# Genie-Kim/PintheMemory

Measured on NVIDIA B200. Metric: memory read+update fwd+bwd Mpixels/s, higher is better.
Workload: dtype f32

## Files before the change

### pinthememory_b200/csrc/pm_gemm.cu

```cuda
#include "pm_common.cuh"
#include "pm_umma.cuh"

namespace pm {

constexpr int GEMM_THREADS = 320;
constexpr int GEMM_RING_BYTES = 192 * 1024;
constexpr int TILE_A_BYTES = 128 * 128;

template <typename T>
struct GemmTraits;
template <>
struct GemmTraits<float> {
    static constexpr int PXC = 32;
    static constexpr int UK = 8;
    static constexpr uint32_t FMT = UMMA_FMT_TF32;
    static constexpr bool SPLIT = true;
};
template <>
struct GemmTraits<__nv_bfloat16> {
    static constexpr int PXC = 64;
    static constexpr int UK = 16;
    static constexpr uint32_t FMT = UMMA_FMT_BF16;
    static constexpr bool SPLIT = false;
};

template <typename T>
__device__ __forceinline__ void umma_issue(uint32_t d, uint64_t a, uint64_t b, uint32_t idesc, uint32_t acc) {
    if constexpr (sizeof(T) == 4) umma_tf32(d, a, b, idesc, acc);
    else umma_bf16(d, a, b, idesc, acc);
}

__device__ __forceinline__ void split_tile_trunc(const float4* __restrict__ raw, float4* __restrict__ lo, int n4, int t,
                                                 int nthreads) {
    for (int i = t; i < n4; i += nthreads) {
        const float4 v = raw[i];
        float4 l;
        l.x = v.x - __uint_as_float(__float_as_uint(v.x) & 0xffffe000u);
        l.y = v.y - __uint_as_float(__float_as_uint(v.y) & 0xffffe000u);
        l.z = v.z - __uint_as_float(__float_as_uint(v.z) & 0xffffe000u);
        l.w = v.w - __uint_as_float(__float_as_uint(v.w) & 0xffffe000u);
        lo[i] = l;
    }
}
__device__ __forceinline__ uint32_t pack_bf16(float a, float b) {
    const __nv_bfloat162 p = __floats2bfloat162_rn(a, b);
    return *reinterpret_cast<const uint32_t*>(&p);
}
__device__ __forceinline__ float tf32_resid(float x) { return x - __uint_as_float(__float_as_uint(x) & 0xffffe000u); }

template <int KB, int NT>
__device__ __forceinline__ void mix_tile_mn(const unsigned char* __restrict__ raw, unsigned char* __restrict__ out, int t,
                                            int nthreads) {
    constexpr int NC32 = NT / 32, ATOMS = KB * NC32 * 4;
    for (int i = t; i < ATOMS; i += nthreads) {
// ... 23 lines not shown
        lo.x = pack_bf16(tf32_resid(v0.x), tf32_resid(v0.y)), lo.y = pack_bf16(tf32_resid(v0.z), tf32_resid(v0.w));
        lo.z = pack_bf16(tf32_resid(v1.x), tf32_resid(v1.y)), lo.w = pack_bf16(tf32_resid(v1.z), tf32_resid(v1.w));
        unsigned char* ro = out + r * 128;
        const int jh = hi_first ? m : 4 + m, jl = hi_first ? 4 + m : m;
        *reinterpret_cast<uint4*>(ro + ((jh ^ (r & 7)) << 4)) = hi;
        *reinterpret_cast<uint4*>(ro + ((jl ^ (r & 7)) << 4)) = lo;
    }
}

__device__ __forceinline__ float tf32_rn(float x) { return __uint_as_float((__float_as_uint(x) + 0x00001000u) & 0xffffe000u); }
__device__ __forceinline__ void split_tile(float4* __restrict__ raw, float4* __restrict__ lo, int n4, int t, int nthreads) {
    for (int i = t; i < n4; i += nthreads) {
        const float4 v = raw[i];
        float4 h, l;
        h.x = tf32_rn(v.x), h.y = tf32_rn(v.y), h.z = tf32_rn(v.z), h.w = tf32_rn(v.w);
        l.x = v.x - h.x, l.y = v.y - h.y, l.z = v.z - h.z, l.w = v.w - h.w;
        lo[i] = l;
        raw[i] = h;
    }
}

struct BnBwdArgs {
    const float *mean, *invstd, *gamma, *beta, *dgamma, *dbeta;
    float inv_n;
    int training, relu;
};

template <int KB>
__device__ __forceinline__ void bnbwd_tile(float4* __restrict__ dy_hi, float4* __restrict__ z_lo, int n4, int t, int nthreads,
                                           int ch0, const BnBwdArgs& bn) {
    constexpr bool FIXED = (KB == 16);
    float is = 0.f, mu = 0.f, sc = 0.f, sh = 0.f, k1 = 0.f, k2 = 0.f;
    auto coef = [&](int c) {
        is = __ldg(bn.invstd + c), mu = __ldg(bn.mean + c);
        sc = is * __ldg(bn.gamma + c), sh = __ldg(bn.beta + c) - mu * sc;
        k1 = bn.training ? __ldg(bn.dbeta + c) * bn.inv_n : 0.f, k2 = bn.training ? __ldg(bn.dgamma + c) * bn.inv_n : 0.f;
    };
    if (FIXED) coef(ch0 + ((t >> 3) % KB));
    for (int i = t; i < n4; i += nthreads) {
        if (!FIXED) coef(ch0 + ((i >> 3) % KB));
        const float4 g = dy_hi[i], z = z_lo[i];
        float4 d, l;
#define PM_BNBWD_ONE(f)                                                                  \
        {                                                                                \
            const float gv = (!bn.relu || fmaf(z.f, sc, sh) > 0.f) ? g.f : 0.f;          \
            const float xh = (z.f - mu) * is;                                            \
            d.f = sc * (gv - k1 - xh * k2);                                              \
            l.f = d.f - __uint_as_float(__float_as_uint(d.f) & 0xffffe000u);             \
        }
        PM_BNBWD_ONE(x) PM_BNBWD_ONE(y) PM_BNBWD_ONE(z) PM_BNBWD_ONE(w)
#undef PM_BNBWD_ONE
        dy_hi[i] = d;
        z_lo[i] = l;
    }
}

template <typename T, int MT, int NT, int KB, int CL, bool MIX>
__global__ void __launch_bounds__(GEMM_THREADS, 1)
    conv1x1_nn_kernel(const __grid_constant__ CUtensorMap mapX, const __grid_constant__ CUtensorMap mapAh,
                      const __grid_constant__ CUtensorMap mapAl, const __grid_constant__ CUtensorMap mapY, int K, int M,
                      int m_tile0, int tiles_per_img, int total_tiles, int accumulate, double* __restrict__ stats,
                      const float* __restrict__ ep_scale, const float* __restrict__ ep_shift, int ep_relu, int dbg,
                      const __grid_constant__ CUtensorMap mapZ, const __grid_constant__ CUtensorMap mapDZ, const BnBwdArgs bn) {
    using TR = GemmTraits<T>;
    constexpr int PXC = TR::PXC, UK = TR::UK, KSTEPS = KB / UK;
    const bool bnbwd = TR::SPLIT && !MIX && bn.mean != nullptr;
    constexpr int NCH = NT / PXC;
    constexpr int XCHUNK = KB * 128;
    constexpr int XBYTES = NCH * XCHUNK;
    constexpr int NOPA = TR::SPLIT ? 2 : 1;
    constexpr int AROW = KB * (int)sizeof(T);
    static_assert(AROW == 128 || AROW == 64, "weight rows must be 64 or 128 bytes");
    constexpr int TILE_A = 128 * AROW;
    constexpr uint32_t ASWZ = AROW == 128 ? UMMA_SW128 : UMMA_SW64, ASBO = 8 * AROW;
    constexpr int STAGE = NOPA * (XBYTES + MT * TILE_A);
    constexpr int STAGES = (GEMM_RING_BYTES / STAGE) > 4 ? 4 : (GEMM_RING_BYTES / STAGE);
    constexpr int ACC = (512 / (MT * NT)) >= 2 ? 2 : 1;
    constexpr uint32_t TX = XBYTES + NOPA * MT * TILE_A;
    static_assert(STAGES >= 2, "ring too small");
    static_assert(MT * NT <= 512, "accumulators exceed TMEM");
    constexpr uint32_t IDESC = umma_idesc(TR::FMT, false, true, 128, NT);
    constexpr uint32_t IDESC_B = umma_idesc(UMMA_FMT_BF16, false, true, 128, NT);
    static_assert(!MIX || (TR::SPLIT && KB % 16 == 0 && NT % 64 == 0), "mixed compensation: fp32 I/O, 16-channel groups");

    extern __shared__ unsigned char smem_raw[];
    unsigned char* smem = smem_align(smem_raw, 1024);
    unsigned char* stg = smem + STAGES * STAGE;
    uint64_t* bars = reinterpret_cast<uint64_t*>(stg + 4 * 2 * 4096);
    uint64_t* full = bars;
    uint64_t* empty = bars + STAGES;
    uint64_t* xfull = bars + 2 * STAGES;
    uint64_t* accf = bars + 3 * STAGES;
    uint64_t* acce = accf + ACC;
    uint64_t* sfree = acce + ACC;
    uint32_t* tmem_slot = reinterpret_cast<uint32_t*>(sfree + STAGES);

    const int warp = threadIdx.x >> 5, lane = threadIdx.x & 31;
    if (threadIdx.x == 0) {
        for (int i = 0; i < STAGES; ++i) {
            mbar_init(&full[i], 1);
            mbar_init(&empty[i], CL);
            mbar_init(&xfull[i], 4);
            mbar_init(&sfree[i], 1);
        }
        for (int i = 0; i < ACC; ++i) {
            mbar_init(&accf[i], 1);
// ... 79 lines not shown
                            const uint64_t ah = umma_desc(sa + mt * TILE_A + ks * 32, 16, ASBO, ASWZ);
                            if (MIX) {
                                umma_issue<T>(d, ah, bh, IDESC, first);
                            } else if (TR::SPLIT) {
                                const uint64_t al = umma_desc(sa + (MT + mt) * TILE_A + ks * 32, 16, ASBO, ASWZ);
                                umma_issue<T>(d, al, bh, IDESC, first);
                                umma_issue<T>(d, ah, bl, IDESC, 1u);
                                umma_issue<T>(d, ah, bh, IDESC, 1u);
                            } else {
                                umma_issue<T>(d, ah, bh, IDESC, first);
                            }
                        }
                    }
                    if (MIX) {
                        const int ksb = 2 * ksteps * UK / 16;
                        for (int ks = 0; ks < ksb; ++ks) {
                            const uint64_t bb = umma_desc(sx + XBYTES + ks * (16 * 128), 2 * KB * 128, 1024, UMMA_SW128);
#pragma unroll
                            for (int mt = 0; mt < MT; ++mt) {
                                const uint32_t d = tmem + (uint32_t)((a * MT + mt) * NT);
                                const uint64_t ab = umma_desc(sa + (MT + mt) * TILE_A + ks * 32, 16, ASBO, ASWZ);
                                umma_bf16(d, ab, bb, IDESC_B, 1u);
                            }
                        }
                    }
                    if (CL == 1) umma_commit(&empty[s]);
                    else umma_commit_multicast(&empty[s], (uint16_t)((1u << CL) - 1));
                }
                umma_commit(&accf[a]);
            }
        }
    } else if (warp < 6) {
        const int q = warp & 3;
        unsigned char* mystg = stg + q * 2 * 4096;
        int bi = 0;
        double sum[MT], sq[MT];
#pragma unroll
        for (int mt = 0; mt < MT; ++mt) sum[mt] = 0.0, sq[mt] = 0.0;
        uint32_t tc = 0;
        for (int g = g0; g < ngroups; g += gstride, ++tc) {
            const int tile = g * CL + crank;
            const int b = tile / tiles_per_img, px0 = (tile - b * tiles_per_img) * NT;
            const int a = tc % ACC;
            mbar_wait(&accf[a], (tc / ACC) & 1);
            tc_fence_after();
#pragma unroll
            for (int mt = 0; mt < MT; ++mt) {
                const int row0 = (m_tile0 + mt) * 128 + q * 32;
                if (row0 >= M || tile >= total_tiles) continue;
                const float sc = ep_scale != nullptr ? __ldg(ep_scale + row0 + lane) : 1.f;
                const float sh = ep_scale != nullptr ? __ldg(ep_shift + row0 + lane) : 0.f;
                float ts = 0.f, tq = 0.f;
                const uint32_t ta0 = tmem + ((uint32_t)(q * 32) << 16) + (uint32_t)((a * MT + mt) * NT);
                auto emit = [&](const uint4 (&out)[8], int c) {
                    unsigned char* buf = mystg + bi * 4096;
                    bi ^= 1;
                    if (lane == 0) bulk_wait_read<1>();
                    __syncwarp();
#pragma unroll
                    for (int j = 0; j < 8; ++j)
                        *reinterpret_cast<uint4*>(buf + lane * 128 + ((j ^ (lane & 7)) << 4)) = out[j];
                    fence_proxy_async_smem();
                    __syncwarp();
                    if (lane == 0) {
                        if (accumulate) tma_reduce_add_2d(&mapY, px0 + c * PXC, b * M + row0, buf);
                        else tma_store_2d(&mapY, px0 + c * PXC, b * M + row0, buf);
                        bulk_commit();
                    }
                };
                if constexpr (sizeof(T) == 4) {
                    auto process = [&](uint32_t (&r)[32], int c) {
                        if (ep_scale != nullptr) {
#pragma unroll
                            for (int j = 0; j < 32; ++j) {
                                float v = fmaf(__uint_as_float(r[j]), sc, sh);
                                if (ep_relu) v = fmaxf(v, 0.f);
                                r[j] = __float_as_uint(v);
                            }
                        }
#pragma unroll
                        for (int j = 0; j < 32; ++j) {
                            const float v = __uint_as_float(r[j]);
                            ts += v;
                            tq = fmaf(v, v, tq);
                        }
                        uint4 out[8];
#pragma unroll
                        for (int j = 0; j < 8; ++j) out[j] = make_uint4(r[4 * j], r[4 * j + 1], r[4 * j + 2], r[4 * j + 3]);
                        emit(out, c);
                    };
                    uint32_t ra[32], rb[32];
                    tmem_ld32(ta0, ra);
#pragma unroll 1
                    for (int c = 0; c < NCH; c += 2) {
                        tmem_ld_wait();
                        if (c + 1 < NCH) tmem_ld32(ta0 + (uint32_t)((c + 1) * PXC), rb);
                        process(ra, c);
                        if (c + 1 < NCH) {
                            tmem_ld_wait();
                            if (c + 2 < NCH) tmem_ld32(ta0 + (uint32_t)((c + 2) * PXC), ra);
                            process(rb, c + 1);
                        }
                    }
                } else {
#pragma unroll 1
                    for (int c = 0; c < NCH; ++c) {
                        const uint32_t ta = ta0 + (uint32_t)(c * PXC);
                        uint4 out[8];
                        uint32_t r0[32], r1[32];
                        tmem_ld32(ta, r0);
                        tmem_ld32(ta + 32, r1);
                        tmem_ld_wait();
                        if (ep_scale != nullptr) {
#pragma unroll
                            for (int j = 0; j < 32; ++j) {
                                float v0 = fmaf(__uint_as_float(r0[j]), sc, sh), v1 = fmaf(__uint_as_float(r1[j]), sc, sh);
                                if (ep_relu) v0 = fmaxf(v0, 0.f), v1 = fmaxf(v1, 0.f);
                                r0[j] = __float_as_uint(v0), r1[j] = __float_as_uint(v1);
                            }
                        }
                        uint32_t pk[32];
#pragma unroll
                        for (int j = 0; j < 16; ++j) {
                            const __nv_bfloat162 p0 = __floats2bfloat162_rn(__uint_as_float(r0[2 * j]), __uint_as_float(r0[2 * j + 1]));
                            const __nv_bfloat162 p1 = __floats2bfloat162_rn(__uint_as_float(r1[2 * j]), __uint_as_float(r1[2 * j + 1]));
                            pk[j] = *reinterpret_cast<const uint32_t*>(&p0);
                            pk[16 + j] = *reinterpret_cast<const uint32_t*>(&p1);
                            const float2 f0 = __bfloat1622float2(p0), f1 = __bfloat1622float2(p1);
                            ts += (f0.x + f0.y) + (f1.x + f1.y);
                            tq = fmaf(f0.x, f0.x, fmaf(f0.y, f0.y, fmaf(f1.x, f1.x, fmaf(f1.y, f1.y, tq))));
                        }
#pragma unroll
                        for (int j = 0; j < 8; ++j) out[j] = make_uint4(pk[4 * j], pk[4 * j + 1], pk[4 * j + 2], pk[4 * j + 3]);
                        emit(out, c);
                    }
                }
                sum[mt] += (double)ts;
                sq[mt] += (double)tq;
            }
            tc_fence_before();
            mbar_arrive(&acce[a]);
        }
        if (lane == 0) bulk_wait<0>();
        if (stats != nullptr) {
#pragma unroll
            for (int mt = 0; mt < MT; ++mt) {
                const int row = (m_tile0 + mt) * 128 + q * 32 + lane;
                if (row < M) {
                    atomicAdd(&stats[row], sum[mt]);
                    atomicAdd(&stats[M + row], sq[mt]);
                }
            }
        }
    } else {
        if constexpr (TR::SPLIT) {
            const int t = threadIdx.x - 6 * 32;
            uint32_t it = 0;
            for (int g = g0; g < ngroups; g += gstride) {
                int tile = g * CL + crank;
                const bool real_tile = tile < total_tiles;
                if (!real_tile) tile = total_tiles - 1;
                const int b = tile / tiles_per_img, px0 = (tile - b * tiles_per_img) * NT;
                for (int kb = 0; kb < nkb; ++kb, ++it) {
                    const int s = it % STAGES;
                    mbar_wait(&full[s], (it / STAGES) & 1);
                    unsigned char* st = smem + s * STAGE;
                    if (MIX) mix_tile_mn<KB, NT>(st, st + XBYTES, t, 128);
                    else if (bnbwd) bnbwd_tile<KB>(reinterpret_cast<float4*>(st), reinterpret_cast<float4*>(st + XBYTES), XBYTES / 16, t, 128, kb * KB, bn);
                    else split_tile_trunc(reinterpret_cast<float4*>(st), reinterpret_cast<float4*>(st + XBYTES), XBYTES / 16, t, 128);
                    fence_proxy_async_smem();
                    __syncwarp();
                    if (lane == 0) mbar_arrive(&xfull[s]);
                    if (bnbwd && t == 0) {
                        mbar_wait(&xfull[s], (it / STAGES) & 1);
                        if (real_tile) {
#pragma unroll
                            for (int c = 0; c < NCH; ++c) tma_store_2d(&mapDZ, px0 + c * PXC, b * K + kb * KB, st + c * XCHUNK);
                        }
                        bulk_commit();
                        bulk_wait_read<1>();
                        if (it > 0) mbar_arrive(&sfree[(it - 1) % STAGES]);
                    }
                }
            }
            if (bnbwd && t == 0) bulk_wait<0>();
        }
    }
// ... 69 lines not shown
    if (!make_map_2d<T>(&mX, X, (size_t)B * K, hw, KB, TR::PXC, sizeof(T) == 4 ? 2 : 1)) return PM_ERR_ALIGN;
    if (!make_map_2d<T>(&mAh, Ah, Mpad, K, 128, KB, ASW)) return PM_ERR_ALIGN;
    const bool mix = TR::SPLIT && gemm_mix() && K % 16 == 0 && bn.mean == nullptr;
    if (mix) {
        if (!make_map_2d<__nv_bfloat16>(&mAl, Al, Mpad, 2 * (size_t)K, 128, 2 * KB, ASW)) return PM_ERR_ALIGN;
    } else if (TR::SPLIT) {
        if (!make_map_2d<T>(&mAl, Al, Mpad, K, 128, KB, ASW)) return PM_ERR_ALIGN;
    } else {
        mAl = mAh;
    }
    if (!make_map_2d<T>(&mY, Y, (size_t)B * M, hw, 32, TR::PXC, true)) return PM_ERR_ALIGN;
    if (bn.mean == nullptr) mZ = mX, mDZ = mX;
    const int tiles_per_img = (hw + NT - 1) / NT, total = B * tiles_per_img;
    const size_t smem = nn_smem_bytes<T, MT, NT, KB>();
    constexpr int NBLK = (TR::SPLIT ? 2 : 1) * MT;
    constexpr int CLMAX = NBLK >= 4 ? 4 : NBLK;
    int cl = gemm_cluster();
    if (cl > CLMAX) cl = CLMAX;
    if (total < 2 * cl) cl = 1;
    cudaLaunchConfig_t cfg{};
    cudaLaunchAttribute attr[1];
    cfg.blockDim = dim3(GEMM_THREADS);
    cfg.dynamicSmemBytes = smem;
    cfg.stream = st;
    attr[0].id = cudaLaunchAttributeClusterDimension;
    attr[0].val.clusterDim.x = cl, attr[0].val.clusterDim.y = 1, attr[0].val.clusterDim.z = 1;
    cfg.attrs = attr, cfg.numAttrs = 1;
    int groups = (total + cl - 1) / cl, clusters = 148 / cl;
    if (clusters > groups) clusters = groups;
    cfg.gridDim = dim3(clusters * cl);
    const int dbg = gemm_dbg();
    cudaError_t e;
#define PM_NN_LAUNCH(CL_)                                                                                             \
    {                                                                                                                 \
        auto kern = mix ? conv1x1_nn_kernel<T, MT, NT, KB, CL_, TR::SPLIT> : conv1x1_nn_kernel<T, MT, NT, KB, CL_, false>; \
        e = cudaFuncSetAttribute(kern, cudaFuncAttributeMaxDynamicSharedMemorySize, (int)smem);                       \
        if (e != cudaSuccess) return (int)e;                                                                          \
        e = cudaLaunchKernelEx(&cfg, kern, mX, mAh, mAl, mY, K, M, m_tile0, tiles_per_img, total, accumulate, stats,     \
                               ep_scale, ep_shift, ep_relu, dbg, mZ, mDZ, bn);                                   \
    }
    if (cl == 4) {
        if constexpr (CLMAX >= 4) PM_NN_LAUNCH(4) else return PM_ERR_SHAPE;
    } else if (cl == 2) {
        if constexpr (CLMAX >= 2) PM_NN_LAUNCH(2) else return PM_ERR_SHAPE;
    } else {
        PM_NN_LAUNCH(1)
    }
#undef PM_NN_LAUNCH
    if (e != cudaSuccess) return (int)e;
    e = cudaGetLastError();
    return e == cudaSuccess ? 0 : (int)e;
}

constexpr int WG_NMAX = 288;

template <typename T, bool MIX>
__global__ void __launch_bounds__(GEMM_THREADS, 1)
    conv1x1_wgrad_kernel(const __grid_constant__ CUtensorMap mapG, const __grid_constant__ CUtensorMap mapX, int M, int N,
                         int Ntot, int n0, int NW, int hw, int chunks_per_img, int blocks_per_chunk, float* __restrict__ part,
                         int Mpad) {
    using TR = GemmTraits<T>;
    constexpr int PXC = TR::PXC, UK = TR::UK, KSTEPS = PXC / UK;
    constexpr int NOPA = TR::SPLIT ? 2 : 1;
    constexpr int BBYTES = WG_NMAX * 128;
    constexpr int STAGE = NOPA * (TILE_A_BYTES + BBYTES);
    constexpr int STAGES = (212992 / STAGE) > 4 ? 4 : (212992 / STAGE);
    static_assert(STAGES >= 2, "ring too small");

    extern __shared__ unsigned char smem_raw[];
    unsigned char* smem = smem_align(smem_raw, 1024);
    uint64_t* bars = reinterpret_cast<uint64_t*>(smem + STAGES * STAGE);
    uint64_t* full = bars;
    uint64_t* empty = bars + STAGES;
    uint64_t* xfull = bars + 2 * STAGES;
    uint64_t* accf = bars + 3 * STAGES;
    uint32_t* tmem_slot = reinterpret_cast<uint32_t*>(accf + 1);

    const int warp = threadIdx.x >> 5, lane = threadIdx.x & 31;
    if (threadIdx.x == 0) {
        for (int i = 0; i < STAGES; ++i) {
            mbar_init(&full[i], 1);
            mbar_init(&empty[i], 1);
            mbar_init(&xfull[i], 4);
        }
        mbar_init(accf, 1);
        asm volatile("fence.mbarrier_init.release.cluster;" ::: "memory");
        prefetch_tmap(&mapG);
        prefetch_tmap(&mapX);
    }
    if (warp == 1) tmem_alloc(tmem_slot, 512);
    tc_fence_before();
    __syncthreads();
    tc_fence_after();
    const uint32_t tmem = *tmem_slot;

    const int chunk = blockIdx.x, mt = blockIdx.y;
    const int b = chunk / chunks_per_img, cb0 = (chunk - b * chunks_per_img) * blocks_per_chunk;
    const int nblk_img = (hw + PXC - 1) / PXC;
    int nkb = nblk_img - cb0;
    if (nkb > blocks_per_chunk) nkb = blocks_per_chunk;
    if (nkb < 0) nkb = 0;
    const int NI = N / NW;
    const uint32_t TX = TILE_A_BYTES + (uint32_t)N * 128;
    const uint32_t IDESC = umma_idesc(TR::FMT, false, false, 128, NW);

    if (warp == 0) {
// ... 233 lines not shown
extern "C" {

int pm_conv1x1_prep_both(const float* W, int R, int S, int dtype, void* A_hi, void* A_lo, void* At_hi, void* At_lo, double* zero,
                         int zero_n, void* stream) {
    if (!W || !A_hi || !At_hi || (dtype == PM_F32 && (!A_lo || !At_lo))) return PM_ERR_NULL;
    if (dtype != PM_F32 && dtype != PM_BF16) return PM_ERR_DTYPE;
    if (R <= 0 || S <= 0 || zero_n < 0 || (zero_n > 0 && !zero)) return PM_ERR_SHAPE;
    const int n0 = (R + 127) / 128 * 128 * S, n1 = (S + 127) / 128 * 128 * R, n = n0 > n1 ? n0 : n1;
    cudaStream_t st = (cudaStream_t)stream;
    const dim3 grid((n + 255) / 256, 2);
    if (dtype == PM_F32)
        conv1x1_prep_both_kernel<float><<<grid, 256, 0, st>>>(W, R, S, (float*)A_hi, (float*)A_lo, (float*)At_hi, (float*)At_lo, gemm_mix(), zero, zero_n);
    else
        conv1x1_prep_both_kernel<__nv_bfloat16><<<grid, 256, 0, st>>>(W, R, S, (__nv_bfloat16*)A_hi, nullptr, (__nv_bfloat16*)At_hi, nullptr, 0, zero, zero_n);
    PM_CHECK_LAUNCH();
    return 0;
}

int pm_conv1x1_prep(const float* W, int M, int K, int transpose, int dtype, void* A_hi, void* A_lo, void* stream) {
    if (!W || !A_hi || (dtype == PM_F32 && !A_lo)) return PM_ERR_NULL;
    if (dtype != PM_F32 && dtype != PM_BF16) return PM_ERR_DTYPE;
    if (M <= 0 || K <= 0) return PM_ERR_SHAPE;
    const int Mpad = (M + 127) / 128 * 128, n = Mpad * K;
    cudaStream_t st = (cudaStream_t)stream;
    if (dtype == PM_F32)
        conv1x1_prep_kernel<float><<<(n + 255) / 256, 256, 0, st>>>(W, M, K, Mpad, transpose, (float*)A_hi, (float*)A_lo,
                                                                    (gemm_mix() && K % 16 == 0) ? 1 : 0);
    else
        conv1x1_prep_kernel<__nv_bfloat16><<<(n + 255) / 256, 256, 0, st>>>(W, M, K, Mpad, transpose, (__nv_bfloat16*)A_hi, nullptr, 0);
    PM_CHECK_LAUNCH();
    return 0;
}

static int conv1x1_fwd_impl(const void* X, const void* A_hi, const void* A_lo, void* Y, double* stats, int B, int K, int M, int hw,
                            int accumulate, const float* ep_scale, const float* ep_shift, int ep_relu, int dtype, void* stream,
                            const void* Z = nullptr, void* DZ = nullptr, const BnBwdArgs* bn = nullptr) {
    if (!X || !A_hi || !Y || (dtype == PM_F32 && !A_lo) || ((ep_scale == nullptr) != (ep_shift == nullptr))) return PM_ERR_NULL;
    if (dtype != PM_F32 && dtype != PM_BF16) return PM_ERR_DTYPE;
    const int esz = dtype == PM_F32 ? 4 : 2, uk = dtype == PM_F32 ? 8 : 16;
    if (B <= 0 || hw <= 0 || K <= 0 || M <= 0 || K % uk || M % 32 || M > 512) return PM_ERR_SHAPE;
    if ((hw * esz) % 16 || ((uintptr_t)X | (uintptr_t)Y | (uintptr_t)A_hi | (uintptr_t)A_lo) % 16) return PM_ERR_ALIGN;
    cudaStream_t st = (cudaStream_t)stream;
    const int Mpad = (M + 127) / 128 * 128, mtiles = Mpad / 128;
    for (int t0 = 0; t0 < mtiles; t0 += 2) {
        const int mt = mtiles - t0 >= 2 ? 2 : 1;
        int rc;
        const bool wide = (long long)B * ((hw + 255) / 256) >= 96;
        if (dtype == PM_F32) {
            const bool first = bn != nullptr && t0 == 0;
            const void* Xin = (bn != nullptr && t0 > 0) ? DZ : X;
            const void* Zi = first ? Z : nullptr;
            void* DZo = first ? DZ : nullptr;
            const BnBwdArgs* bi = first ? bn : nullptr;
            if (wide && !gemm_narrow())
                rc = mt == 2 ? launch_nn<float, 2, 256, 16>(Xin, A_hi, A_lo, Y, stats, B, K, M, Mpad, hw, t0, accumulate, ep_scale, ep_shift, ep_relu, st, Zi, DZo, bi)
                             : launch_nn<float, 1, 256, 16>(Xin, A_hi, A_lo, Y, stats, B, K, M, Mpad, hw, t0, accumulate, ep_scale, ep_shift, ep_relu, st, Zi, DZo, bi);
            else
                rc = mt == 2 ? launch_nn<float, 2, 128, 32>(Xin, A_hi, A_lo, Y, stats, B, K, M, Mpad, hw, t0, accumulate, ep_scale, ep_shift, ep_relu, st, Zi, DZo, bi)
                             : launch_nn<float, 1, 128, 32>(Xin, A_hi, A_lo, Y, stats, B, K, M, Mpad, hw, t0, accumulate, ep_scale, ep_shift, ep_relu, st, Zi, DZo, bi);
        } else {
            rc = mt == 2 ? launch_nn<__nv_bfloat16, 2, 128, 64>(X, A_hi, A_lo, Y, stats, B, K, M, Mpad, hw, t0, accumulate, ep_scale, ep_shift, ep_relu, st)
                         : launch_nn<__nv_bfloat16, 1, 128, 64>(X, A_hi, A_lo, Y, stats, B, K, M, Mpad, hw, t0, accumulate, ep_scale, ep_shift, ep_relu, st);
        }
        if (rc) return rc;
    }
    return 0;
}

int pm_conv1x1_fwd(const void* X, const void* A_hi, const void* A_lo, void* Y, double* stats, int B, int K, int M, int hw,
                   int accumulate, int dtype, void* stream) {
    return conv1x1_fwd_impl(X, A_hi, A_lo, Y, stats, B, K, M, hw, accumulate, nullptr, nullptr, 0, dtype, stream);
}

int pm_conv1x1_dgrad_bnbwd(const void* dY, const void* Z, const void* A_hi, const void* A_lo, void* dX, void* dZ,
                           const float* mean, const float* invstd, const float* gamma, const float* beta, const float* dgamma,
                           const float* dbeta, int relu, int training, int B, int K, int M, int hw, int dtype, void* stream) {
    if (!Z || !dZ || !mean || !invstd || !gamma || !beta || !dgamma || !dbeta) return PM_ERR_NULL;
    if (dtype != PM_F32) return PM_ERR_DTYPE;
    if (K % 32 || ((uintptr_t)Z | (uintptr_t)dZ) % 16) return PM_ERR_ALIGN;
    BnBwdArgs bn{mean, invstd, gamma, beta, dgamma, dbeta, 1.f / ((float)B * (float)hw), training, relu};
    return conv1x1_fwd_impl(dY, A_hi, A_lo, dX, nullptr, B, K, M, hw, 0, nullptr, nullptr, 0, dtype, stream, Z, dZ, &bn);
}

int pm_conv1x1_fwd_affine(const void* X, const void* A_hi, const void* A_lo, void* Y, const float* scale, const float* shift,
                          int relu, int B, int K, int M, int hw, int dtype, void* stream) {
    if (!scale || !shift) return PM_ERR_NULL;
    return conv1x1_fwd_impl(X, A_hi, A_lo, Y, nullptr, B, K, M, hw, 0, scale, shift, relu, dtype, stream);
}

int pm_conv1x1_wgrad_workspace_floats(int B, int M, int N, int hw, int dtype) {
    if (B <= 0 || M <= 0 || N <= 0 || hw <= 0) return 0;
    int cpi, bpc;
    wgrad_split(B, M, hw, dtype == PM_F32 ? 32 : 64, &cpi, &bpc);
    const int Mpad = (M + 127) / 128 * 128;
    const int nmax = N > WG_NMAX ? WG_NMAX : N;
    return B * cpi * Mpad * nmax;
}

int pm_conv1x1_wgrad(const void* dY, const void* X, float* workspace, float* dW, int B, int M, int N, int hw, int accumulate,
                     int dtype, void* stream) {
    if (!dY || !X || !workspace || !dW) return PM_ERR_NULL;
    if (dtype != PM_F32 && dtype != PM_BF16) return PM_ERR_DTYPE;
    const int esz = dtype == PM_F32 ? 4 : 2;
    if (B <= 0 || hw <= 0 || M <= 0 || N <= 0 || M % 32 || N % 32 || M > 512 || N > 1024) return PM_ERR_SHAPE;
    if ((hw * esz) % 16 || ((uintptr_t)X | (uintptr_t)dY | (uintptr_t)workspace | (uintptr_t)dW) % 16) return PM_ERR_ALIGN;
    cudaStream_t st = (cudaStream_t)stream;
    for (int n0 = 0; n0 < N;) {
// ... 12 lines not shown
```

### pinthememory_b200/csrc/pm_umma.cuh

```cuda
#pragma once
#include "pm_tma.cuh"

namespace pm {

__device__ __forceinline__ void mbar_arrive(uint64_t* bar) {
    asm volatile("mbarrier.arrive.shared::cta.b64 _, [%0];" ::"r"(smem_u32(bar)) : "memory");
}
__device__ __forceinline__ void fence_proxy_async_smem() { asm volatile("fence.proxy.async.shared::cta;" ::: "memory"); }
__device__ __forceinline__ void tc_fence_before() { asm volatile("tcgen05.fence::before_thread_sync;" ::: "memory"); }
__device__ __forceinline__ void tc_fence_after() { asm volatile("tcgen05.fence::after_thread_sync;" ::: "memory"); }

__device__ __forceinline__ void tmem_alloc(uint32_t* smem_dst, uint32_t ncols) {
    asm volatile("tcgen05.alloc.cta_group::1.sync.aligned.shared::cta.b32 [%0], %1;" ::"r"(smem_u32(smem_dst)), "r"(ncols)
                 : "memory");
    asm volatile("tcgen05.relinquish_alloc_permit.cta_group::1.sync.aligned;" ::: "memory");
}
__device__ __forceinline__ void tmem_dealloc(uint32_t taddr, uint32_t ncols) {
    asm volatile("tcgen05.dealloc.cta_group::1.sync.aligned.b32 %0, %1;" ::"r"(taddr), "r"(ncols) : "memory");
}

constexpr uint32_t UMMA_SW128 = 2, UMMA_SW128_BASE32B = 1, UMMA_SW64 = 4;
__device__ __forceinline__ uint64_t umma_desc(uint32_t saddr, uint32_t lbo_bytes, uint32_t sbo_bytes,
                                              uint32_t layout = UMMA_SW128) {
    uint64_t d = (uint64_t)((saddr & 0x3FFFFu) >> 4);
// ... 1 lines not shown
    d |= (uint64_t)((sbo_bytes >> 4) & 0x3FFFu) << 32;
    d |= (uint64_t)1 << 46;
    d |= (uint64_t)layout << 61;
    return d;
}

constexpr uint32_t UMMA_FMT_BF16 = 1, UMMA_FMT_TF32 = 2;
__host__ __device__ constexpr uint32_t umma_idesc(uint32_t fmt, bool a_mn_major, bool b_mn_major, int M, int N) {
    return (1u << 4) | (fmt << 7) | (fmt << 10) | ((a_mn_major ? 1u : 0u) << 15) | ((b_mn_major ? 1u : 0u) << 16) |
           ((uint32_t)(N >> 3) << 17) | ((uint32_t)(M >> 4) << 24);
}

__device__ __forceinline__ void umma_tf32(uint32_t d_tmem, uint64_t adesc, uint64_t bdesc, uint32_t idesc, uint32_t acc) {
    asm volatile(
        "{\n.reg .pred p;\nsetp.ne.b32 p, %4, 0;\n"
        "tcgen05.mma.cta_group::1.kind::tf32 [%0], %1, %2, %3, p;\n}" ::"r"(d_tmem),
        "l"(adesc), "l"(bdesc), "r"(idesc), "r"(acc)
        : "memory");
}
__device__ __forceinline__ void umma_bf16(uint32_t d_tmem, uint64_t adesc, uint64_t bdesc, uint32_t idesc, uint32_t acc) {
    asm volatile(
        "{\n.reg .pred p;\nsetp.ne.b32 p, %4, 0;\n"
        "tcgen05.mma.cta_group::1.kind::f16 [%0], %1, %2, %3, p;\n}" ::"r"(d_tmem),
        "l"(adesc), "l"(bdesc), "r"(idesc), "r"(acc)
        : "memory");
}
__device__ __forceinline__ void umma_commit(uint64_t* bar) {
    asm volatile("tcgen05.commit.cta_group::1.mbarrier::arrive::one.shared::cluster.b64 [%0];" ::"r"(smem_u32(bar)) : "memory");
}

__device__ __forceinline__ void umma_commit_multicast(uint64_t* bar, uint16_t cta_mask) {
    asm volatile("tcgen05.commit.cta_group::1.mbarrier::arrive::one.shared::cluster.multicast::cluster.b64 [%0], %1;" ::"r"(
                     smem_u32(bar)),
                 "h"(cta_mask)
                 : "memory");
}
__device__ __forceinline__ void tma_load_2d_multicast(void* dst, const CUtensorMap* map, int c0, int c1, uint64_t* bar,
                                                      uint16_t cta_mask) {
    asm volatile(
        "cp.async.bulk.tensor.2d.shared::cluster.global.tile.mbarrier::complete_tx::bytes.multicast::cluster [%0], [%1, {%2, "
        "%3}], [%4], %5;" ::"r"(smem_u32(dst)),
        "l"(reinterpret_cast<uint64_t>(map)), "r"(c0), "r"(c1), "r"(smem_u32(bar)), "h"(cta_mask)
        : "memory");
}
__device__ __forceinline__ uint32_t cluster_ctarank() {
    uint32_t r;
    asm volatile("mov.u32 %0, %%cluster_ctarank;" : "=r"(r));
    return r;
}
__device__ __forceinline__ void cluster_sync_all() {
    asm volatile("barrier.cluster.arrive.release.aligned;\nbarrier.cluster.wait.acquire.aligned;" ::: "memory");
}

__device__ __forceinline__ void tmem_ld32(uint32_t taddr, uint32_t (&r)[32]) {
    asm volatile(
        "tcgen05.ld.sync.aligned.32x32b.x32.b32 "
        "{%0, %1, %2, %3, %4, %5, %6, %7, %8, %9, %10, %11, %12, %13, %14, %15, "
        "%16, %17, %18, %19, %20, %21, %22, %23, %24, %25, %26, %27, %28, %29, %30, %31}, [%32];"
        : "=r"(r[0]), "=r"(r[1]), "=r"(r[2]), "=r"(r[3]), "=r"(r[4]), "=r"(r[5]), "=r"(r[6]), "=r"(r[7]), "=r"(r[8]),
          "=r"(r[9]), "=r"(r[10]), "=r"(r[11]), "=r"(r[12]), "=r"(r[13]), "=r"(r[14]), "=r"(r[15]), "=r"(r[16]),
          "=r"(r[17]), "=r"(r[18]), "=r"(r[19]), "=r"(r[20]), "=r"(r[21]), "=r"(r[22]), "=r"(r[23]), "=r"(r[24]),
          "=r"(r[25]), "=r"(r[26]), "=r"(r[27]), "=r"(r[28]), "=r"(r[29]), "=r"(r[30]), "=r"(r[31])
        : "r"(taddr)
        : "memory");
}
__device__ __forceinline__ void tmem_ld_wait() { asm volatile("tcgen05.wait::ld.sync.aligned;" ::: "memory"); }

__device__ __forceinline__ void tma_store_2d(const CUtensorMap* map, int c0, int c1, const void* src) {
    asm volatile("cp.async.bulk.tensor.2d.global.shared::cta.bulk_group [%0, {%2, %3}], [%1];" ::"l"(
                     reinterpret_cast<uint64_t>(map)),
                 "r"(smem_u32(src)), "r"(c0), "r"(c1)
                 : "memory");
}
__device__ __forceinline__ void tma_reduce_add_2d(const CUtensorMap* map, int c0, int c1, const void* src) {
    asm volatile("cp.reduce.async.bulk.tensor.2d.global.shared::cta.add.bulk_group [%0, {%2, %3}], [%1];" ::"l"(
                     reinterpret_cast<uint64_t>(map)),
                 "r"(smem_u32(src)), "r"(c0), "r"(c1)
                 : "memory");
}
__device__ __forceinline__ void bulk_commit() { asm volatile("cp.async.bulk.commit_group;" ::: "memory"); }
template <int N>
__device__ __forceinline__ void bulk_wait_read() {
    asm volatile("cp.async.bulk.wait_group.read %0;" ::"n"(N) : "memory");
}
template <int N>
__device__ __forceinline__ void bulk_wait() {
    asm volatile("cp.async.bulk.wait_group %0;" ::"n"(N) : "memory");
}
__device__ __forceinline__ void prefetch_tmap(const CUtensorMap* map) {
    asm volatile("prefetch.tensormap [%0];" ::"l"(reinterpret_cast<uint64_t>(map)) : "memory");
}

}
```

Baseline: 92.29.

## Add 2-CTA paired UMMA kernel for fused BN-backward conv1x1 with M=256

Adds a cluster-of-two kernel that issues tcgen05 cta_group::2 TF32 MMAs (256x256 tiles) for the first-K-block BN-backward split-precision conv1x1 path when two M tiles are present. The two CTAs share each other's X/Z tiles, run the BN backward transform and write dZ in-CTA, and coordinate through cross-CTA mbarriers. The goal is to halve B-operand loading per M tile and increase MMA tile size. The f32 epilogue is factored into shared helpers with a pixel-bound check. This adds synchronisation complexity and a new occupancy-dependent launch path.

Result: faster. 93.81 (median of 6 runs) (+1.6%).

```diff
diff --git a/pinthememory_b200/csrc/pm_gemm.cu b/pinthememory_b200/csrc/pm_gemm.cu
--- a/pinthememory_b200/csrc/pm_gemm.cu
+++ b/pinthememory_b200/csrc/pm_gemm.cu
@@ -1,5 +1,6 @@
 #include "pm_common.cuh"
 #include "pm_umma.cuh"
+
 
 namespace pm {
 
@@ -129,6 +130,61 @@
 #undef PM_BNBWD_ONE
         dy_hi[i] = d;
         z_lo[i] = l;
+    }
+}
+
+__device__ __forceinline__ void ep_emit(const uint4 (&out)[8], unsigned char* mystg, int& bi, int lane, const CUtensorMap* mapY,
+                                        int x, int y, int accumulate) {
+    unsigned char* buf = mystg + bi * 4096;
+    bi ^= 1;
+    if (lane == 0) bulk_wait_read<1>();
+    __syncwarp();
+#pragma unroll
+    for (int j = 0; j < 8; ++j) *reinterpret_cast<uint4*>(buf + lane * 128 + ((j ^ (lane & 7)) << 4)) = out[j];
+    fence_proxy_async_smem();
+    __syncwarp();
+    if (lane == 0) {
+        if (accumulate) tma_reduce_add_2d(mapY, x, y, buf);
+        else tma_store_2d(mapY, x, y, buf);
+        bulk_commit();
+    }
+}
+__device__ __forceinline__ void ep_rows_f32(uint32_t ta0, int nch, unsigned char* mystg, int& bi, int lane, const CUtensorMap* mapY,
+                                            int x0, int xend, int y, int accumulate, bool affine, float sc, float sh, int relu,
+                                            float& ts, float& tq) {
+    auto process = [&](uint32_t (&r)[32], int c) {
+        if (affine) {
+#pragma unroll
+            for (int j = 0; j < 32; ++j) {
+                float v = fmaf(__uint_as_float(r[j]), sc, sh);
+                if (relu) v = fmaxf(v, 0.f);
+                r[j] = __float_as_uint(v);
+            }
+        }
+#pragma unroll
+        for (int j = 0; j < 32; ++j) {
+            const float v = __uint_as_float(r[j]);
+            ts += v;
+            tq = fmaf(v, v, tq);
+        }
+        if (x0 + c * 32 >= xend) return;
+        uint4 out[8];
+#pragma unroll
+        for (int j = 0; j < 8; ++j) out[j] = make_uint4(r[4 * j], r[4 * j + 1], r[4 * j + 2], r[4 * j + 3]);
+        ep_emit(out, mystg, bi, lane, mapY, x0 + c * 32, y, accumulate);
+    };
+    uint32_t ra[32], rb[32];
+    tmem_ld32(ta0, ra);
+#pragma unroll 1
+    for (int c = 0; c < nch; c += 2) {
+        tmem_ld_wait();
+        if (c + 1 < nch) tmem_ld32(ta0 + (uint32_t)((c + 1) * 32), rb);
+        process(ra, c);
+        if (c + 1 < nch) {
+            tmem_ld_wait();
+            if (c + 2 < nch) tmem_ld32(ta0 + (uint32_t)((c + 2) * 32), ra);
+            process(rb, c + 1);
+        }
     }
 }
 
@@ -314,56 +370,9 @@
                 const float sh = ep_scale != nullptr ? __ldg(ep_shift + row0 + lane) : 0.f;
                 float ts = 0.f, tq = 0.f;
                 const uint32_t ta0 = tmem + ((uint32_t)(q * 32) << 16) + (uint32_t)((a * MT + mt) * NT);
-                auto emit = [&](const uint4 (&out)[8], int c) {
-                    unsigned char* buf = mystg + bi * 4096;
-                    bi ^= 1;
-                    if (lane == 0) bulk_wait_read<1>();
-                    __syncwarp();
-#pragma unroll
-                    for (int j = 0; j < 8; ++j)
-                        *reinterpret_cast<uint4*>(buf + lane * 128 + ((j ^ (lane & 7)) << 4)) = out[j];
-                    fence_proxy_async_smem();
-                    __syncwarp();
-                    if (lane == 0) {
-                        if (accumulate) tma_reduce_add_2d(&mapY, px0 + c * PXC, b * M + row0, buf);
-                        else tma_store_2d(&mapY, px0 + c * PXC, b * M + row0, buf);
-                        bulk_commit();
-                    }
-                };
                 if constexpr (sizeof(T) == 4) {
-                    auto process = [&](uint32_t (&r)[32], int c) {
-                        if (ep_scale != nullptr) {
-#pragma unroll
-                            for (int j = 0; j < 32; ++j) {
-                                float v = fmaf(__uint_as_float(r[j]), sc, sh);
-                                if (ep_relu) v = fmaxf(v, 0.f);
-                                r[j] = __float_as_uint(v);
-                            }
-                        }
-#pragma unroll
-                        for (int j = 0; j < 32; ++j) {
-                            const float v = __uint_as_float(r[j]);
-                            ts += v;
-                            tq = fmaf(v, v, tq);
-                        }
-                        uint4 out[8];
-#pragma unroll
-                        for (int j = 0; j < 8; ++j) out[j] = make_uint4(r[4 * j], r[4 * j + 1], r[4 * j + 2], r[4 * j + 3]);
-                        emit(out, c);
-                    };
-                    uint32_t ra[32], rb[32];
-                    tmem_ld32(ta0, ra);
-#pragma unroll 1
-                    for (int c = 0; c < NCH; c += 2) {
-                        tmem_ld_wait();
-                        if (c + 1 < NCH) tmem_ld32(ta0 + (uint32_t)((c + 1) * PXC), rb);
-                        process(ra, c);
-                        if (c + 1 < NCH) {
-                            tmem_ld_wait();
-                            if (c + 2 < NCH) tmem_ld32(ta0 + (uint32_t)((c + 2) * PXC), ra);
-                            process(rb, c + 1);
-                        }
-                    }
+                    ep_rows_f32(ta0, NCH, mystg, bi, lane, &mapY, px0, INT_MAX, b * M + row0, accumulate, ep_scale != nullptr, sc, sh,
+                                ep_relu, ts, tq);
                 } else {
 #pragma unroll 1
                     for (int c = 0; c < NCH; ++c) {
@@ -394,7 +403,7 @@
                         }
 #pragma unroll
                         for (int j = 0; j < 8; ++j) out[j] = make_uint4(pk[4 * j], pk[4 * j + 1], pk[4 * j + 2], pk[4 * j + 3]);
-                        emit(out, c);
+                        ep_emit(out, mystg, bi, lane, &mapY, px0 + c * PXC, b * M + row0, accumulate);
                     }
                 }
                 sum[mt] += (double)ts;
@@ -570,6 +579,216 @@
     return e == cudaSuccess ? 0 : (int)e;
 }
 
+constexpr int PAIR_NP = 256;
+constexpr int PAIR_STAGE = 2 * (PAIR_NP * 16 * 4 + 128 * 16 * 4);
+constexpr int PAIR_STAGES = GEMM_RING_BYTES / PAIR_STAGE;
+
+__global__ void __launch_bounds__(GEMM_THREADS, 1)
+    conv1x1_pair_bnbwd_kernel(const __grid_constant__ CUtensorMap mapX, const __grid_constant__ CUtensorMap mapAh,
+                              const __grid_constant__ CUtensorMap mapAl, const __grid_constant__ CUtensorMap mapY, int K, int M,
+                              int hw, int m_tile0, int tiles_per_img, int total_tiles, const __grid_constant__ CUtensorMap mapZ,
+                              const __grid_constant__ CUtensorMap mapDZ, const BnBwdArgs bn) {
+    constexpr int PXC = 32, UK = 8, KB = 16, KSTEPS = KB / UK;
+    constexpr int NCH = PAIR_NP / PXC;
+    constexpr int XCHUNK = KB * 128;
+    constexpr int XBYTES = NCH * XCHUNK;
+    constexpr int TILE_A = 128 * KB * 4;
+    constexpr int STAGES = PAIR_STAGES;
+    constexpr uint32_t TX = 2 * XBYTES + 2 * TILE_A;
+    constexpr uint32_t IDESC = umma_idesc(UMMA_FMT_TF32, false, true, 256, 256);
+    static_assert(XBYTES + XBYTES + 2 * TILE_A == PAIR_STAGE && STAGES >= 2, "pair ring layout");
+
+    extern __shared__ unsigned char smem_raw[];
+    unsigned char* smem = smem_align(smem_raw, 1024);
+    unsigned char* stg = smem + STAGES * PAIR_STAGE;
+    uint64_t* bars = reinterpret_cast<uint64_t*>(stg + 4 * 2 * 4096);
+    uint64_t* full = bars;
+    uint64_t* empty = bars + STAGES;
+    uint64_t* xfull = bars + 2 * STAGES;
+    uint64_t* xpair = bars + 3 * STAGES;
+    uint64_t* sfree = bars + 4 * STAGES;
+    uint64_t* accf = bars + 5 * STAGES;
+    uint64_t* acce = accf + 1;
+    uint32_t* tmem_slot = reinterpret_cast<uint32_t*>(acce + 1);
+
+    const int warp = threadIdx.x >> 5, lane = threadIdx.x & 31;
+    const uint32_t rank = cluster_ctarank();
+    if (threadIdx.x == 0) {
+        for (int i = 0; i < STAGES; ++i) {
+            mbar_init(&full[i], 1);
+            mbar_init(&empty[i], 1);
+            mbar_init(&xfull[i], 4);
+            mbar_init(&xpair[i], 8);
+            mbar_init(&sfree[i], 1);
+        }
+        mbar_init(accf, 1);
+        mbar_init(acce, 256);
+        asm volatile("fence.mbarrier_init.release.cluster;" ::: "memory");
+        prefetch_tmap(&mapX);
+        prefetch_tmap(&mapAh);
+        prefetch_tmap(&mapY);
+    }
+    if (warp == 1) tmem_alloc_pair(tmem_slot, 512);
+    tc_fence_before();
+    __syncthreads();
+    cluster_sync_all();
+    tc_fence_after();
+    const uint32_t tmem = *tmem_slot;
+    const int nkb = K / KB;
+    const int g0 = blockIdx.x / 2, gstride = gridDim.x / 2;
+    auto chunk_px = [&](int c) { return 256 * (c / 4) + 128 * (int)rank + PXC * (c % 4); };
+
+    if (warp == 0) {
+        if (lane == 0) {
+            uint32_t it = 0;
+            for (int g = g0; g < total_tiles; g += gstride) {
+                const int b = g / tiles_per_img, px0 = (g - b * tiles_per_img) * 2 * PAIR_NP;
+                for (int kb = 0; kb < nkb; ++kb, ++it) {
+                    const int s = it % STAGES;
+                    mbar_wait(&empty[s], ((it / STAGES) & 1) ^ 1);
+                    mbar_wait(&sfree[s], ((it / STAGES) & 1) ^ 1);
+                    unsigned char* st = smem + s * PAIR_STAGE;
+                    mbar_expect_tx(&full[s], TX);
+#pragma unroll
+                    for (int c = 0; c < NCH; ++c) {
+                        tma_load_2d(st + c * XCHUNK, &mapX, px0 + chunk_px(c), b * K + kb * KB, &full[s]);
+                        tma_load_2d(st + XBYTES + c * XCHUNK, &mapZ, px0 + chunk_px(c), b * K + kb * KB, &full[s]);
+                    }
+                    unsigned char* sa = st + 2 * XBYTES;
+                    tma_load_2d(sa, &mapAh, kb * KB, (m_tile0 + (int)rank) * 128, &full[s]);
+                    tma_load_2d(sa + TILE_A, &mapAl, kb * KB, (m_tile0 + (int)rank) * 128, &full[s]);
+                }
+            }
+        }
+    } else if (warp == 1) {
+        if (lane == 0 && rank == 0) {
+            uint32_t it = 0, tc = 0;
+            for (int g = g0; g < total_tiles; g += gstride, ++tc) {
+                mbar_wait(acce, (tc & 1) ^ 1);
+                tc_fence_after();
+                for (int kb = 0; kb < nkb; ++kb, ++it) {
+                    const int s = it % STAGES;
+                    mbar_wait(&xpair[s], (it / STAGES) & 1);
+                    tc_fence_after();
+                    const uint32_t sx = smem_u32(smem + s * PAIR_STAGE);
+                    const uint32_t sa = sx + 2 * XBYTES;
+#pragma unroll
+                    for (int ks = 0; ks < KSTEPS; ++ks) {
+                        const uint64_t ah = umma_desc(sa + ks * 32, 16, 8 * 64, UMMA_SW64);
+                        const uint64_t al = umma_desc(sa + TILE_A + ks * 32, 16, 8 * 64, UMMA_SW64);
+                        const uint32_t first = (kb | ks) ? 1u : 0u;
+#pragma unroll
+                        for (int j = 0; j < 2; ++j) {
+                            const uint32_t bx = sx + j * 4 * XCHUNK + ks * (UK * 128);
+                            const uint64_t bh = umma_desc(bx, XCHUNK, 512, UMMA_SW128_BASE32B);
+                            const uint64_t bl = umma_desc(bx + XBYTES, XCHUNK, 512, UMMA_SW128_BASE32B);
+                            const uint32_t d = tmem + (uint32_t)(j * 256);
+                            umma_tf32_pair(d, al, bh, IDESC, first);
+                            umma_tf32_pair(d, ah, bl, IDESC, 1u);
+                            umma_tf32_pair(d, ah, bh, IDESC, 1u);
+                        }
+                    }
+                    umma_commit_pair_multicast(&empty[s], 0x3);
+                }
+                umma_commit_pair_multicast(accf, 0x3);
+            }
+        }
+    } else if (warp < 6) {
+        const int q = warp & 3;
+        unsigned char* mystg = stg + q * 2 * 4096;
+        int bi = 0;
+        const int row0 = (m_tile0 + (int)rank) * 128 + q * 32;
+        const uint32_t acce0 = cluster_addr(acce, 0);
+        uint32_t tc = 0;
+        for (int g = g0; g < total_tiles; g += gstride, ++tc) {
+            const int b = g / tiles_per_img, px0 = (g - b * tiles_per_img) * 2 * PAIR_NP;
+            mbar_wait(accf, tc & 1);
+            tc_fence_after();
+            if (row0 < M) {
+                float ts = 0.f, tq = 0.f;
+                ep_rows_f32(tmem + ((uint32_t)(q * 32) << 16), 2 * NCH, mystg, bi, lane, &mapY, px0, hw, b * M + row0, 0, false,
+                            1.f, 0.f, 0, ts, tq);
+            }
+            tc_fence_before();
+            mbar_arrive_cluster(acce0);
+        }
+        if (lane == 0) bulk_wait<0>();
+    } else {
+        const int t = threadIdx.x - 6 * 32;
+        const uint32_t xpair0 = cluster_addr(xpair, 0);
+        uint32_t it = 0;
+        for (int g = g0; g < total_tiles; g += gstride) {
+            const int b = g / tiles_per_img, px0 = (g - b * tiles_per_img) * 2 * PAIR_NP;
+            for (int kb = 0; kb < nkb; ++kb, ++it) {
+                const int s = it % STAGES;
+                mbar_wait(&full[s], (it / STAGES) & 1);
+                unsigned char* st = smem + s * PAIR_STAGE;
+                bnbwd_tile<KB>(reinterpret_cast<float4*>(st), reinterpret_cast<float4*>(st + XBYTES), XBYTES / 16, t, 128, kb * KB, bn);
+                fence_proxy_async_smem();
+                __syncwarp();
+                if (lane == 0) {
+                    mbar_arrive_cluster(xpair0 + (uint32_t)(s * 8));
+                    mbar_arrive(&xfull[s]);
+                }
+                if (t == 0) {
+                    mbar_wait(&xfull[s], (it / STAGES) & 1);
+#pragma unroll
+                    for (int c = 0; c < NCH; ++c)
+                        if (px0 + chunk_px(c) < hw) tma_store_2d(&mapDZ, px0 + chunk_px(c), b * K + kb * KB, st + c * XCHUNK);
+                    bulk_commit();
+                    bulk_wait_read<1>();
+                    if (it > 0) mbar_arrive(&sfree[(it - 1) % STAGES]);
+                }
+            }
+        }
+        if (t == 0) bulk_wait<0>();
+    }
+    tc_fence_before();
+    __syncthreads();
+    cluster_sync_all();
+    if (warp == 1) {
+        tc_fence_after();
+        tmem_dealloc_pair(tmem, 512);
+    }
+}
+
+static int launch_pair_bnbwd(const void* X, const void* Ah, const void* Al, void* Y, int B, int K, int M, int Mpad, int hw,
+                             int m_tile0, cudaStream_t st, const void* Z, void* DZ, const BnBwdArgs& bn) {
+    if (K % 16 != 0) return PM_ERR_SHAPE;
+    CUtensorMap mX, mAh, mAl, mY, mZ, mDZ;
+    if (!make_map_2d<float>(&mX, X, (size_t)B * K, hw, 16, 32, 2)) return PM_ERR_ALIGN;
+    if (!make_map_2d<float>(&mZ, Z, (size_t)B * K, hw, 16, 32, 2)) return PM_ERR_ALIGN;
+    if (!make_map_2d<float>(&mDZ, DZ, (size_t)B * K, hw, 16, 32, 2)) return PM_ERR_ALIGN;
+    if (!make_map_2d<float>(&mAh, Ah, Mpad, K, 128, 16, 3)) return PM_ERR_ALIGN;
+    if (!make_map_2d<float>(&mAl, Al, Mpad, K, 128, 16, 3)) return PM_ERR_ALIGN;
+    if (!make_map_2d<float>(&mY, Y, (size_t)B * M, hw, 32, 32, 1)) return PM_ERR_ALIGN;
+    const int tiles_per_img = (hw + 2 * PAIR_NP - 1) / (2 * PAIR_NP), total = B * tiles_per_img;
+    const size_t smem = (size_t)PAIR_STAGES * PAIR_STAGE + 4 * 2 * 4096 + 512 + 1024;
+    cudaLaunchConfig_t cfg{};
+    cudaLaunchAttribute attr[1];
+    cfg.gridDim = dim3(2);
+    cfg.blockDim = dim3(GEMM_THREADS);
+    cfg.dynamicSmemBytes = smem;
+    cfg.stream = st;
+    attr[0].id = cudaLaunchAttributeClusterDimension;
+    attr[0].val.clusterDim.x = 2, attr[0].val.clusterDim.y = 1, attr[0].val.clusterDim.z = 1;
+    cfg.attrs = attr, cfg.numAttrs = 1;
+    auto kern = conv1x1_pair_bnbwd_kernel;
+    cudaError_t e = cudaFuncSetAttribute(kern, cudaFuncAttributeMaxDynamicSharedMemorySize, (int)smem);
+    if (e != cudaSuccess) return (int)e;
+    static const int max_pairs = [&] {
+        int n = 0;
+        return cudaOccupancyMaxActiveClusters(&n, kern, &cfg) == cudaSuccess ? n : 0;
+    }();
+    if (max_pairs < 1) return PM_ERR_SHAPE;
+    const int pairs = max_pairs < total ? max_pairs : total;
+    cfg.gridDim = dim3(2 * pairs);
+    e = cudaLaunchKernelEx(&cfg, kern, mX, mAh, mAl, mY, K, M, hw, m_tile0, tiles_per_img, total, mZ, mDZ, bn);
+    if (e != cudaSuccess) return (int)e;
+    e = cudaGetLastError();
+    return e == cudaSuccess ? 0 : (int)e;
+}
+
 constexpr int WG_NMAX = 288;
 
 template <typename T, bool MIX>
@@ -909,7 +1128,9 @@
             const void* Zi = first ? Z : nullptr;
             void* DZo = first ? DZ : nullptr;
             const BnBwdArgs* bi = first ? bn : nullptr;
-            if (wide && !gemm_narrow())
+            if (first && wide && mt == 2 && !gemm_narrow())
+                rc = launch_pair_bnbwd(X, A_hi, A_lo, Y, B, K, M, Mpad, hw, t0, st, Z, DZ, *bn);
+            else if (wide && !gemm_narrow())
                 rc = mt == 2 ? launch_nn<float, 2, 256, 16>(Xin, A_hi, A_lo, Y, stats, B, K, M, Mpad, hw, t0, accumulate, ep_scale, ep_shift, ep_relu, st, Zi, DZo, bi)
                              : launch_nn<float, 1, 256, 16>(Xin, A_hi, A_lo, Y, stats, B, K, M, Mpad, hw, t0, accumulate, ep_scale, ep_shift, ep_relu, st, Zi, DZo, bi);
             else
diff --git a/pinthememory_b200/csrc/pm_umma.cuh b/pinthememory_b200/csrc/pm_umma.cuh
--- a/pinthememory_b200/csrc/pm_umma.cuh
+++ b/pinthememory_b200/csrc/pm_umma.cuh
@@ -77,6 +77,36 @@
     asm volatile("barrier.cluster.arrive.release.aligned;\nbarrier.cluster.wait.acquire.aligned;" ::: "memory");
 }
 
+__device__ __forceinline__ void tmem_alloc_pair(uint32_t* smem_dst, uint32_t ncols) {
+    asm volatile("tcgen05.alloc.cta_group::2.sync.aligned.shared::cta.b32 [%0], %1;" ::"r"(smem_u32(smem_dst)), "r"(ncols)
+                 : "memory");
+    asm volatile("tcgen05.relinquish_alloc_permit.cta_group::2.sync.aligned;" ::: "memory");
+}
+__device__ __forceinline__ void tmem_dealloc_pair(uint32_t taddr, uint32_t ncols) {
+    asm volatile("tcgen05.dealloc.cta_group::2.sync.aligned.b32 %0, %1;" ::"r"(taddr), "r"(ncols) : "memory");
+}
+__device__ __forceinline__ void umma_tf32_pair(uint32_t d_tmem, uint64_t adesc, uint64_t bdesc, uint32_t idesc, uint32_t acc) {
+    asm volatile(
+        "{\n.reg .pred p;\nsetp.ne.b32 p, %4, 0;\n"
+        "tcgen05.mma.cta_group::2.kind::tf32 [%0], %1, %2, %3, p;\n}" ::"r"(d_tmem),
+        "l"(adesc), "l"(bdesc), "r"(idesc), "r"(acc)
+        : "memory");
+}
+__device__ __forceinline__ void umma_commit_pair_multicast(uint64_t* bar, uint16_t cta_mask) {
+    asm volatile("tcgen05.commit.cta_group::2.mbarrier::arrive::one.shared::cluster.multicast::cluster.b64 [%0], %1;" ::"r"(
+                     smem_u32(bar)),
+                 "h"(cta_mask)
+                 : "memory");
+}
+__device__ __forceinline__ uint32_t cluster_addr(const void* p, uint32_t rank) {
+    uint32_t r;
+    asm volatile("mapa.shared::cluster.u32 %0, %1, %2;" : "=r"(r) : "r"(smem_u32(p)), "r"(rank));
+    return r;
+}
+__device__ __forceinline__ void mbar_arrive_cluster(uint32_t bar_cluster_addr) {
+    asm volatile("mbarrier.arrive.shared::cluster.b64 _, [%0];" ::"r"(bar_cluster_addr) : "memory");
+}
+
 __device__ __forceinline__ void tmem_ld32(uint32_t taddr, uint32_t (&r)[32]) {
     asm volatile(
         "tcgen05.ld.sync.aligned.32x32b.x32.b32 "
```
